# Iasonaspg/GPU-Randomized-Block-Lanczos

Hardware: AMD Instinct MI355X
Metric: RBL iters/sec + time-to-k=20 eigenpairs, n=1e7 nnz/row=100 b=32; 1/2/4/8 GPU (higher is better)
Workload: dtype f64

## Files before the change

gpu-randomized-block-lanczos_amd/csrc/kernels.hpp:

```cpp
#pragma once
#include "rbl_common.hpp"

namespace rbl {

struct Panels {
  static constexpr int kMax = 2;
  const double* ptr[kMax] = {nullptr, nullptr};
  int count = 0;
  int w = 0;
};
struct PanelRun {
  const double* base = nullptr;
  const float* base32 = nullptr;
  int64_t stride = 0;
  int count = 0;
  int w = 0;
};

constexpr int64_t kCsrPad = 256;
constexpr int64_t kRowPad = 16;
constexpr int64_t kRowPad32 = 32;

struct CsrDev {
  int64_t nrows = 0;
// ... 194 lines not shown
  double* beta = nullptr;
  double* bb = nullptr;
  double* rr = nullptr;
  int* iters = nullptr;
  int* status = nullptr;
  int* nactive = nullptr;
  double* hist = nullptr;
};
int cg_grid(int64_t nrows, int b);
void cg_resid(int64_t nrows, int b, const double* B, const double* W, const double* X, double sigma,
              double* R, double* part, double* dots, hipStream_t s);
void cg_dot(int64_t nrows, int b, const double* P, const double* W, double sigma, double* part,
            double* dots, hipStream_t s);
void cg_alpha(int b, const double* pap, const CgScalars& sc, hipStream_t s);
void cg_update(int64_t nrows, int b, double* X, double* R, const double* P, const double* W, double sigma,
               const CgScalars& sc, double* part, double* dots, hipStream_t s);
void cg_small(int rp, int b, const double* dv, const double* w, double* c, hipStream_t s);
void cg_beta(int b, int rp, bool init, int iter, const double* dots, const double* w, const double* c,
             double tol2, const CgScalars& sc, hipStream_t s);
void cg_dir(int64_t nrows, int b, int rp, const double* R, double* P, const double* V, const double* c,
            const CgScalars& sc, hipStream_t s);

constexpr int kKernRbf = 0, kKernLaplace = 1, kKernPoly = 2;
constexpr int kKernMaxDim = 256;
struct KernOp {
  int64_t n = 0;
  int d4 = 0;
  int kind = kKernRbf;
  int degree = 1;
  double gamma = 1.0, coef0 = 0.0, nugget = 0.0;
  const double* X = nullptr;
  const double* nrm = nullptr;
  const double* scale = nullptr;
};
void kernop_norms(int64_t n, int d4, const double* X, double* nrm, hipStream_t s);
bool kernop_apply(const KernOp& op, const double* Q, int b, double* U, hipStream_t s);

struct KernCross {
  int64_t mr = 0, mc = 0;
  int d4 = 0;
  int kind = kKernRbf;
  int degree = 1;
  double gamma = 1.0, coef0 = 0.0;
  const double* R = nullptr;
  const double* rnrm = nullptr;
  const double* C = nullptr;
  const double* cnrm = nullptr;
  const double* sr = nullptr;
  const double* sc = nullptr;
};
constexpr int kKernCrossWorkgroups = 512, kKernCrossMaxSplits = 64, kKernCrossMinStages = 4;
int kernop_cross_splits(int64_t mr, int64_t mc, int d4);
bool kernop_cross(const KernCross& op, const double* W, int b, double* Y, double* part, int splits,
                  hipStream_t s);

int gram_splits(int64_t nrows, int nW, int w, int xcols);
void gram_partial(int64_t nrows, const PanelRun& W, const Panels& X, double* slab, int splits,
                  const int* skip, hipStream_t s);
void reduce_slab(const double* slab, int splits, int64_t len, double* out, const int* skip,
                 hipStream_t s);
int reduce_scratch_splits(int splits);
void reduce_slab_many(double* slab, int splits, int64_t len, double* out, hipStream_t s);
void tsmm(int64_t nrows, const PanelRun& X, const double* C, int ldc, const Panels& Y,
          double alpha, double beta, const int* skip, hipStream_t s, double* xslab = nullptr,
          int* xgrid = nullptr);

constexpr int kCompressMaxCols = 512;
bool basis_compress_fast(const PanelRun& X, int p);
bool basis_compress(int64_t nrows, const PanelRun& X, const double* S_dev, int p, hipStream_t s,
                    bool generic = false);

bool gram44_ok(int64_t nrows, int nW, int w, int xcount, int xw);
int gram44_splits(int64_t nrows, int nW, int w = 32);
void gram44_partial(int64_t nrows, const PanelRun& W, const Panels& X, double* slab, int splits,
                    const int* skip, hipStream_t s);
bool tsmm44_ok(int xw, int ky, int yw);
void tsmm44_f32x(int64_t nrows, const PanelRun& X, const double* C, int ldc, const Panels& Y,
                 double alpha, double beta, hipStream_t s);
int tsmm44_xg_grid(int64_t nrows);
void tsmm44(int64_t nrows, const PanelRun& X, const double* C, int ldc, const Panels& Y,
            double alpha, double beta, const int* skip, hipStream_t s, double* xslab = nullptr,
            int* xgrid = nullptr);
bool tsmm44x32_ok(int64_t nrows, const PanelRun& X, const Panels& Y);
void tsmm44x32(int64_t nrows, const PanelRun& X, const double* C, int ldc, const Panels& Y,
               const int* skip, hipStream_t s);
int64_t tsmm44x32_shadow_slot(int64_t nrows);
void tsmm44x32_shadow(int64_t nrows, const PanelRun& X, const double* C, int ldc, const Panels& Y,
                      const int* skip, float* S, int nsh, int* cnt, hipStream_t s);
void shadow_block_rowmajor(const float* slot, int64_t nrows, float* out);

int gram32_splits(int64_t nrows);
void gram32_partial(int64_t nrows, const float* Wb, int64_t wstride, int nW, int w, const float* X0,
                    const float* X1, int xcount, double* slab, int splits, hipStream_t s);
void tsmm32(int64_t nrows, const float* Xb, int64_t xstride, int nX, int w, const double* C, int ldc,
            float* Y0, float* Y1, int ycount, float alpha, float beta, hipStream_t s);
void cvt_f32_to_f64(const float* src, double* dst, int64_t n, hipStream_t s);
void cvt_f64_to_f32(const double* src, float* dst, int64_t n, hipStream_t s);

void chol_step(const double* G, int b, int64_t nglobal, int mode, double* R, double* Rinv,
               double* Rtot, int* need3, int* status, const int* skip, hipStream_t s,
               double* scratch);
void copy_small(const double* src, double* dst, int64_t len, hipStream_t s, const int* skip = nullptr);
void cloc_rinv(double* C, const double* Rinv, int b, const int* skip, hipStream_t s);
void cloc_rinv2(double* C, const double* R1inv, const double* R2inv, int b, hipStream_t s);
void cloc_gate(const double* R, const double* Rinv, int b, const int* need3, double tau, int* gate,
               hipStream_t s);
void upd32_gate(const double* C, int K, int ncols, double tau, int force, int* flags, double* g_out,
                hipStream_t s);
void cloc_sub(double* G, const double* D, int nW, int b, hipStream_t s);
void transpose_small(const double* src, double* dst, int b, hipStream_t s);
void stash_step(const double* Ai, const double* Rtot, double* Bprev, int* flags, double* stash,
                int b, hipStream_t s);

struct RmatParams {
  int64_t n = 0;
  int scale = 0;
  int64_t edges = 0;
  double a = 0.57, b = 0.19, c = 0.19;
  uint64_t seed = 0;
  bool relabel = false;
  Scatter perm;
};
constexpr uint64_t kRelabelK = 0x52454C4142454C31ull;
void rmat_degree(const RmatParams& p, int32_t* deg, hipStream_t s);
int rmat_local_csr(const RmatParams& p, int64_t r0, int64_t r1, int64_t max_keys, int nplant,
                   const double* plant_dev, int64_t* rowptr_dev, int32_t** col_dev,
                   double** val_dev, int64_t* nnz_out, hipStream_t s);
void col_footprint(const int32_t* col, int64_t nnz, const int64_t* bounds_dev, int P,
                   unsigned long long* lo, unsigned long long* hi, hipStream_t s);

void circ_count(int64_t n, int64_t width, double p, uint64_t seed, int64_t r0, int64_t r1,
                int32_t* counts, hipStream_t s);
void circ_fill(int64_t n, int64_t width, double p, uint64_t seed, int64_t r0, int64_t r1,
               const int64_t* rowptr, int nplant, const double* plant_dev, int32_t* col,
               double* val, hipStream_t s);
void gather_rows(const double* Q, const int32_t* idx, int64_t nrows, int b, double* out,
                 hipStream_t s);
void mark_cols(const int32_t* col, int64_t nnz, int64_t r0, int64_t r1, uint8_t* mark,
               hipStream_t s);
void remap_cols(int32_t* col, int64_t nnz, const int32_t* map, hipStream_t s);
void hw_count(int64_t n, int64_t W, double p, uint64_t seed, int64_t r0, int64_t r1,
              int32_t* counts, hipStream_t s);
void hw_fill(int64_t n, int64_t W, double p, uint64_t seed, int64_t r0, int64_t r1,
             const int64_t* rowptr, int nplant, const double* plant_dev, int32_t* col,
             double* val, hipStream_t s);
void randn_block(double* Q, int64_t nrows, int b, int64_t r0, uint64_t seed, hipStream_t s,
                 const Scatter* perm = nullptr);
void tile_col_range(const CsrDev& A, int tile_rows, int64_t* cmin, int64_t* cmax, hipStream_t s);
void colmajor_to_rowmajor(const double* src, int64_t nrows, int w, double* dst, hipStream_t s);
void rowmajor_to_colmajor(const double* src, int64_t nrows, int w, double* dst, hipStream_t s);

}
```

gpu-randomized-block-lanczos_amd/csrc/rbl_api.cpp:

```cpp
#include <hip/hip_runtime.h>
#include <rocprofiler-sdk-roctx/roctx.h>

#include <algorithm>
#include <cstdlib>
#include <chrono>
#include <cmath>
#include <cstdio>
#include <cstring>
#include <string>
#include <thread>
#include <vector>

#include "../../include/rbl_hip.h"
#include "comm.hpp"
#include "kernels.hpp"

using namespace rbl;

namespace rbl::api {

template <class T>
struct DevBuf {
  T* p = nullptr;
  DevBuf() = default;
// ... 73 lines not shown
  DevBuf<int32_t> d_panel_blk;
  DevBuf<uint16_t> d_panel_cnt;
  DevBuf<uint32_t> d_panel_st;
  DevBuf<uint8_t> d_panel_col;
  DevBuf<double> d_panel_val;
};

struct SegTableBufs {
  DevBuf<int64_t> d_seg_trow;
  DevBuf<int32_t> d_seg_tinfo;
  DevBuf<int64_t> d_seg_slot_k0;
  DevBuf<int64_t> d_seg_lrow;
  DevBuf<int64_t> d_seg_lslot;
  DevBuf<double> d_seg_scratch;
};

struct TierBufs {
  SegTierBuf seg_tier[3];
  DevBuf<int32_t> d_send_idx;
  SegTierBuf push_tier;
  DevBuf<int64_t> d_ps_rows;
  DevBuf<int64_t> d_ps_ptr;
  DevBuf<int64_t> d_ps_slot;
};

struct RectShiftBufs {
  DevBuf<double> d_shift_u;
  DevBuf<double> d_shift_v;
  DevBuf<double> d_rect_ts;
  DevBuf<double> d_rect_part;
};

struct LowrankBufs {
  DevBuf<double> d_lr_P;
  DevBuf<double> d_lr_S;
  DevBuf<double> d_lr_wc;
  DevBuf<double> d_lr_part;
};

struct PrecondBufs {
  DevBuf<double> d_pc_V;
  DevBuf<double> d_pc_dv;
};

struct MatrixBufs : PanelBufs, SegTableBufs, TierBufs, RectShiftBufs, LowrankBufs, PrecondBufs {
  DevBuf<int64_t> d_rowptr;
  DevBuf<int32_t> d_col;
  DevBuf<double> d_val;
  DevBuf<int64_t> d_tcmin;
  DevBuf<int64_t> d_tcmax;
  DevBuf<int64_t> d_tinfo;
  DevBuf<uint16_t> d_bpos;
  DevBuf<double> d_bt;
  DevBuf<uint64_t> d_btp_hdr;
  DevBuf<double> d_bth;
  DevBuf<double> d_bte;
  DevBuf<double> d_btp_val;
  DevBuf<double> d_zrow;
  DevBuf<double> d_dense;
  DevBuf<double> d_qfull;
  SegTierBuf rect_side[2];
  DevBuf<double> d_rect_y;
  DevBuf<double> d_kern_x;
  DevBuf<double> d_kern_nrm;
  DevBuf<double> d_kern_scale;
};

struct RunBufs {
  DevBuf<double> d_basis;
  std::vector<PinBuf<char>> h_spill;
  DevBuf<double> d_stage;
  DevBuf<float> d_basis32;
  DevBuf<float> d_stage32;
  DevBuf<double> d_Qi64;
  DevBuf<double> d_Qm64;
  DevBuf<double> d_U;
  DevBuf<double> d_T;
  DevBuf<double> d_qext;
  DevBuf<double> d_sendbuf;
  DevBuf<double> d_pushbuf;
  DevBuf<double> d_precv;
  DevBuf<double> d_slab;
  DevBuf<double> d_C;
  DevBuf<double> d_small;
  DevBuf<int> d_flags;
  PinBuf<double> h_pin;
  PinBuf<double> h_hist;
  DevBuf<double> d_stash;
  DevBuf<double> d_lock;
  DevBuf<double> d_arrow_W;
  DevBuf<double> d_tr_S;
  DevBuf<double> d_filt[3];
  DevBuf<double> d_rv;
  DevBuf<double> d_rw;
  DevBuf<float> d_shadow;
};

struct CtxBufs {
  PinBuf<char> h_d2h[2];
  DevBuf<int> d_upd32;
  DevBuf<double> d_upd32_g;
};

}

struct rbl_ctx : rbl::api::MatrixBufs, rbl::api::RunBufs, rbl::api::CtxBufs {
  int device = 0;
  hipStream_t stream = nullptr;
  int nranks = 1, rank = 0;
  rbl::Comm* comm = nullptr;
  std::string err;

  int64_t n = 0, r0 = 0, r1 = 0, nloc = 0, nnz = 0;
  int64_t panel_nblk = 0;
  int panel_rpg = 4;
  int panel_ch = 48;
  bool panel_auto = false;
  int64_t panel_span = 0;
  int bt_ng = 0;
  int64_t seg_ntasks = 0, seg_nlong = 0;
  int seg_ntiers = 0;
  bool seg_split = false;
  bool ghost = false;
  int64_t n_ghost = 0, n_send = 0;
  std::vector<int64_t> ghost_cnt, ghost_off, send_cnt, send_off;
  const double* ghost_local = nullptr;
  bool ghost_active = false;
  bool halo_overlap = true;
  int halo_push_opt = 2;
  bool push = false;
  int64_t push_rows = 0;
  int64_t n_ps_rows = 0;
  size_t push_cap = 0;
  int64_t push_pred_rows = 0, pull_pred_rows = 0;
  hipEvent_t ev_push_ready = nullptr, ev_push_done = nullptr;
  hipStream_t hstream = nullptr;
  hipEvent_t ev_qready = nullptr, ev_halo = nullptr;
  bool dense = false;
  int64_t dense_panels = 0;
  int qfull_cols = 0;
  bool rect = false;
  int64_t rect_m = 0;
  int rect_y_cols = 0;
  bool rect_shift = false;
  int rect_ts_cols = 0;
  bool kernop = false;
  int kern_d = 0, kern_d4 = 0, kern_kind = 0, kern_degree = 0;
  double kern_gamma = 0.0, kern_coef0 = 0.0, kern_nugget = 0.0;
  int lr_r = 0, lr_rp = 0;
  int lr_cols = 0;
  int pc_r = 0, pc_rp = 0;
  int64_t ntiles = 0, tiles_per_wg = 0;
  bool window_ok16 = false, window_ok32 = false;
  bool band_ok16 = false, band_ok32 = false;
  bool band_gram = false;
  bool band_pair = false;
  std::vector<int64_t> bounds;
  std::vector<int64_t> need_lo, need_hi;
  std::vector<int64_t> give_lo, give_hi;
  int64_t ext_lo = 0, ext_hi = 0;
  bool split_halo = true;
  bool keep_csr = true;
  int relabel_opt = 0;
  bool relabeled = false;
  rbl::Scatter relabel_perm;
  bool csr_dropped = false;
// ... 1375 lines not shown
  const double c = 0.5 * (ctx->ser_lo + ctx->ser_hi), e = 0.5 * (ctx->ser_hi - ctx->ser_lo);
  const double* t1 = X;
  const double* t2 = nullptr;
  const int64_t len = ctx->nloc * b;
  for (int j = 1; j <= d; ++j) {
    double* tj = F[j % 3];
    const int st = apply_A(ctx, t1, 0, b, tj, nullptr, nullptr, nullptr);
    if (st < 0) return st;
    const double al = (j == 1 ? 1.0 : 2.0) / e;
    cheb_series_term(len, tj, t1, t2, al, -al * c, mu[j], mu[0], tj, out, j == 1, j == d, ctx->stream);
    HIPC(hipGetLastError());
    t2 = t1;
    t1 = tj;
  }
  return RBL_OK;
}

int filter_apply(rbl_ctx* ctx, const double* X, int b, double* out, const DevBuf<double> F[3]) {
  if (has_series(ctx)) return series_apply(ctx, X, b, out, F);
  return cheb_apply(ctx, X, b, out, F[0], F[1]);
}

constexpr double kUpd32Tau = 0.5;
constexpr int kUpd32Log = 64;

int lock_reorth(rbl_ctx* ctx, double* X) {
  const int b = ctx->b;
  for (int j = 0; j < ctx->nlock; ++j) {
    const double* l = ctx->d_lock + (int64_t)j * ctx->nloc;
    CHK(gram(ctx, run1(l, 1), pan1(X, b), ctx->d_C, nullptr));
    CHK(tsmm_checked(ctx, run1(l, 1), ctx->d_C, b, pan1(X, b), -1.0, 1.0, nullptr));
  }
  return RBL_OK;
}

bool cloc_derive_on(const rbl_ctx* ctx) {
  return ctx->cloc_derive && ctx->basis_bits == 64 && rowgram_ok(ctx->b) && (ctx->fuse & 3) == 3 &&
         ctx->reorth_order == 0 && !spilled(ctx) && (ctx->nranks == 1 || ctx->plan_all_resident);
}

int reorth_pair(rbl_ctx* ctx, int i, int flags) {
  const int b = ctx->b;
  double* Qi = slotp(ctx, i - 1);
  double* Qm = i >= 2 ? slotp(ctx, i - 2) : nullptr;
  shadow_written(ctx, i - 2);
  if ((flags & 2) && ctx->nlock > 0) {
    StageScope t(ctx, RBL_STAGE_PART_REORTH);
    if (Qm) CHK(lock_reorth(ctx, Qm));
    CHK(lock_reorth(ctx, Qi));
  }
  if ((flags & 1) && i >= 3) {
    StageScope t(ctx, RBL_STAGE_PART_REORTH);
    const int nW = i - 2;
    const int nres = std::min(nW, ctx->resident);
    const bool derive = cloc_derive_on(ctx) && b == 32 && ctx->cloc_step == i && !ctx->cloc_final &&
                        !((flags & 2) && ctx->nlock > 0) && nres == nW;
    const bool xg = (ctx->fuse & 2) && b == 32 && !derive;
    const int xg_parts = tsmm44_xg_grid(ctx->nloc);
    const bool xslab_ok = (size_t)(xg_parts + reduce_scratch_splits(xg_parts)) * b * b <= ctx->slab_elems;
    int xgrid = 0;
    auto update = [&](const PanelRun& W, bool last) -> int {
      const bool here = xg && last && xslab_ok;
      return tsmm_checked(ctx, W, ctx->d_C, 2 * b, pan2(Qi, Qm, b), -1.0, 1.0, nullptr,
                          here ? ctx->d_slab : nullptr, here ? &xgrid : nullptr);
    };
    if (ctx->reorth_order == 0) {
      PanelRun W;
      W.base = slotp(ctx, 0);
      W.stride = ctx->slot;
      W.count = nres;
      W.w = b;
      CHK(gram(ctx, W, pan2(Qi, Qm, b), ctx->d_C, nullptr));
      const Panels Yp = pan2(Qi, Qm, b);
      const bool gate32 = ctx->upd32 != 0 && b == 32 && !xg && nres == nW && !((flags & 2) && ctx->nlock > 0);
      const bool u32 = gate32 && ctx->nloc > 0 && tsmm44x32_ok(ctx->nloc, W, Yp);
      if (gate32) {
        upd32_gate(ctx->d_C, nW * b, 2 * b, kUpd32Tau, ctx->upd32 == 2, ctx->d_upd32,
                   ctx->d_upd32_g + (i % kUpd32Log), ctx->stream);
        HIPC(hipGetLastError());
      }
      if (u32) {
        if (ctx->d_shadow && ctx->shadow_opt && nW <= ctx->max_blocks - 2) {
          tsmm44x32_shadow(ctx->nloc, W, ctx->d_C, 2 * b, Yp, ctx->d_upd32, ctx->d_shadow,
                           ctx->shadow_valid, ctx->d_upd32 + 4, ctx->stream);
          ctx->shadow_valid = nW;
        } else {
          tsmm44x32(ctx->nloc, W, ctx->d_C, 2 * b, Yp, ctx->d_upd32, ctx->stream);
        }
        HIPC(hipGetLastError());
        CHK(tsmm_checked(ctx, W, ctx->d_C, 2 * b, Yp, -1.0, 1.0, ctx->d_upd32 + 1));
      } else {
        CHK(update(W, nres == nW));
      }
    } else {
      for (int j = 0; j < nres; ++j) {
        const PanelRun W = run1(slotp(ctx, j), b);
        CHK(gram(ctx, W, pan2(Qi, Qm, b), ctx->d_C, nullptr));
        CHK(update(W, j == nW - 1));
      }
    }
    for (int j = nres; j < nW; ++j) {
      int st = 0;
      const double* Wj = block_dev(ctx, j, i, &st);
      if (st) return fail(ctx, st, "partial reorth: H2D of a spilled block failed");
      CHK(gram(ctx, run1(Wj, b), pan2(Qi, Qm, b), ctx->d_C, nullptr));
      CHK(update(run1(Wj, b), j == nW - 1));
    }
    if (xg) {
      if (xgrid > 0) {
        reduce_slab_many(ctx->d_slab, xgrid, (int64_t)b * b, smallp(ctx, S_CLOC), ctx->stream);
      } else if (ctx->nloc > 0) {
        const int sp = gram_splits(ctx->nloc, 1, b, b);
        gram_partial(ctx->nloc, run1(Qm, b), pan1(Qi, b), ctx->d_slab, sp, nullptr, ctx->stream);
        reduce_slab(ctx->d_slab, sp, (int64_t)b * b, smallp(ctx, S_CLOC), nullptr, ctx->stream);
      } else {
        HIPC(hipMemsetAsync(smallp(ctx, S_CLOC), 0, (size_t)b * b * sizeof(double), ctx->stream));
      }
      HIPC(hipGetLastError());
      CHK(allreduce(ctx, smallp(ctx, S_CLOC), (size_t)b * b));
      ctx->cloc_step = i;
      ctx->cloc_final = true;
      ctx->cloc_src = 0;
    }
    if (derive) {
      cloc_sub(smallp(ctx, S_CLOC), ctx->d_C, nW, b, ctx->stream);
      HIPC(hipGetLastError());
      ctx->cloc_final = true;
      ctx->cloc_src = 2;
    }
  }
  return RBL_OK;
}

int combine_blocks(rbl_ctx* ctx, int nblocks, int kcols, const double* d_S, double* Y) {
  const int b = ctx->b;
  const int nres = std::min(nblocks, ctx->resident);
  PanelRun X;
  X.base = slotp(ctx, 0);
  X.stride = ctx->slot;
  X.count = nres;
  X.w = b;
  CHK(tsmm_checked(ctx, X, d_S, kcols, pan1(Y, kcols), 1.0, 0.0, nullptr));
  for (int j = nres; j < nblocks; ++j) {
    int st = 0;
    const double* Qj = block_dev(ctx, j, ctx->nblocks, &st);
    if (st) return fail(ctx, st, "Ritz: H2D of a spilled block failed");
    CHK(tsmm_checked(ctx, run1(Qj, b), d_S + (int64_t)j * b * kcols, kcols, pan1(Y, kcols), 1.0,
                     1.0, nullptr));
  }
  return RBL_OK;
}

int basis_combine(rbl_ctx* ctx, int nblocks, int kcols, const double* S, double* Y) {
  const int b = ctx->b;
  const int64_t rows = (int64_t)nblocks * b;
  DevBuf<double> d_Scm, d_S;
  HIPC(d_Scm.alloc(rows * kcols));
  HIPC(d_S.alloc(rows * kcols));
  HIPC(hipMemcpyAsync(d_Scm, S, rows * kcols * sizeof(double), hipMemcpyHostToDevice, ctx->stream));
  colmajor_to_rowmajor(d_Scm, rows, kcols, d_S, ctx->stream);
  const int st = combine_blocks(ctx, nblocks, kcols, d_S, Y);
  HIPC(hipStreamSynchronize(ctx->stream));
  return st;
}

int combine_blocks32(rbl_ctx* ctx, int nblocks, int kcols, const double* d_S, double* Y) {
  const int b = ctx->b;
  if (ctx->nloc <= 0) return RBL_OK;
  const int nres = std::min(nblocks, ctx->resident);
  int j0 = 0;
// ... 1663 lines not shown
  HIPC(hipSetDevice(ctx->device));
  HIPC(hipStreamSynchronize(ctx->stream));
  int dev_slots = max_blocks + 1;
  const bool same_shape = (ctx->d_basis || ctx->d_basis32) && ctx->b == b &&
                          ctx->max_blocks == max_blocks && ctx->slot == ctx->nloc * b &&
                          ctx->basis_bits == basis_bits;
  const int cur_slots = ctx->resident == INT32_MAX ? ctx->max_blocks + 1 : ctx->resident + 2;
  if (ctx->dev_blocks_opt < 0 && same_shape && ctx->auto_planned) {
    dev_slots = cur_slots;
  } else if (ctx->dev_blocks_opt != 0) {
    int g = ctx->dev_blocks_opt;
    if (g < 0) {
      size_t fr = 0, tot = 0;
      HIPC(hipMemGetInfo(&fr, &tot));
      const double blk64 = (double)std::max<int64_t>(ctx->nloc, 1) * b * 8.0;
      const double blk = blk64 * (basis_bits == 64 ? 1.0 : 0.5);
      const double mine = ctx->d_basis ? (double)(ctx->resident == INT32_MAX ? ctx->max_blocks + 1 : ctx->resident + 2) * blk64
                        : ctx->d_basis32 ? (double)(ctx->resident == INT32_MAX ? ctx->max_blocks + 1 : ctx->resident + 2) * blk64 * 0.5
                        : 0.0;
      const double mine_all = mine + (double)ctx->shadow_bytes;
      const double work = 2.0 + (ctx->nranks > 1 ? 1.0 : 0.0) +
                          (basis_bits == 32 ? 1.0 + (direct32_ok(ctx, b) ? 0.0 : 1.0) : 0.0);
      const double other = work * blk64 + blk + 8.0 * (double)gram_slab_elems(ctx, b, max_blocks, basis_bits);
      g = (int)std::max(3.0, std::floor((0.8 * ((double)fr + mine_all) - other) / blk));
    }
    dev_slots = std::min(dev_slots, std::max(3, g));
  }
  const bool reuse = same_shape && cur_slots == dev_slots;
  ctx->plan_all_resident = ctx->dev_blocks_opt == 0;
  ctx->nlock = 0;
  ctx->arrow_kb = 0;
  ctx->cloc_step = 0;
  ctx->shadow_valid = 0;
  ctx->step_flags.clear();
  const int alloc_st = [&]() -> int {
  if (reuse) {
    ctx->nblocks = 0;
    if (ctx->cstream) HIPC(hipStreamSynchronize(ctx->cstream));
    ctx->d2h_pending[0] = ctx->d2h_pending[1] = false;
    HIPC(hipMemsetAsync(ctx->d_flags, 0, 4 * sizeof(int), ctx->stream));
  } else {
  free_run(ctx);
  ctx->b = b;
  ctx->max_blocks = max_blocks;
  ctx->slot = ctx->nloc * b;
  const int64_t nl = std::max<int64_t>(ctx->nloc, 1);
  ctx->basis_bits = basis_bits;
  ctx->auto_planned = ctx->dev_blocks_opt < 0;
  if (basis_bits == 64) {
    HIPC(ctx->d_basis.alloc((size_t)dev_slots * nl * b));
    if (dev_slots < max_blocks + 1) {
      ctx->resident = dev_slots - 2;
      ctx->h_spill = std::vector<PinBuf<char>>(max_blocks + 1 - ctx->resident);
      HIPC(ctx->d_stage.alloc((size_t)nl * b));
      CHK(ensure_spill_stream(ctx));
    }
  } else {
    const size_t len32 = ((size_t)dev_slots * nl + kRowPad32) * b;
    HIPC(ctx->d_basis32.alloc(len32));
    HIPC(hipMemsetAsync(ctx->d_basis32, 0, len32 * sizeof(float), ctx->stream));
    if (dev_slots < max_blocks + 1) {
      ctx->resident = dev_slots - 2;
      ctx->h_spill = std::vector<PinBuf<char>>(max_blocks + 1 - ctx->resident);
      HIPC(ctx->d_stage32.alloc(((size_t)nl + kRowPad32) * b));
      HIPC(hipMemsetAsync(ctx->d_stage32, 0, ((size_t)nl + kRowPad32) * b * sizeof(float), ctx->stream));
      CHK(ensure_spill_stream(ctx));
    }
    HIPC(ctx->d_Qi64.alloc((nl + kRowPad) * b));
    if (!direct32_ok(ctx, b)) HIPC(ctx->d_Qm64.alloc((nl + kRowPad) * b));
  }
  HIPC(ctx->d_U.alloc((nl + kRowPad) * b));
  ctx->T_cols = b;
  HIPC(ctx->d_T.alloc(nl * b));
  if (ctx->nranks > 1) {
    CHK(ensure_qext(ctx, b, ctx->stream));
    if (ctx->ghost)
      HIPC(ctx->d_sendbuf.alloc(std::max<int64_t>(ctx->n_send, 1) * b));
  }
  const size_t slab = gram_slab_elems(ctx, b, max_blocks, basis_bits);
  ctx->slab_elems = slab;
  HIPC(ctx->d_slab.alloc(slab));
  ctx->C_elems = (size_t)std::max(1, max_blocks) * b * 2 * b;
  HIPC(ctx->d_C.alloc(ctx->C_elems));
  HIPC(ctx->d_small.alloc((size_t)S_NSMALL * b * b));
  HIPC(hipMemset(ctx->d_small, 0, (size_t)S_NSMALL * b * b * sizeof(double)));
  HIPC(ctx->d_flags.alloc(6));
  HIPC(hipMemset(ctx->d_flags, 0, 6 * sizeof(int)));
  if (!ctx->d_upd32) {
    HIPC(ctx->d_upd32.alloc(6));
    HIPC(hipMemset(ctx->d_upd32, 0, 6 * sizeof(int)));
    HIPC(ctx->d_upd32_g.alloc(kUpd32Log));
    HIPC(hipMemset(ctx->d_upd32_g, 0, kUpd32Log * sizeof(double)));
  }
  {
#ifdef RBL_VARIANTS
    const char* e = std::getenv("RBL_STASH_COPY");
    ctx->stash_direct = !(e && std::atoi(e) == 1);
#else
    ctx->stash_direct = true;
#endif
    const unsigned hf = ctx->stash_direct ? (hipHostMallocMapped | hipHostMallocCoherent) : hipHostMallocDefault;
    HIPC(ctx->h_pin.alloc(stash_rec(b), hf));
    HIPC(ctx->h_hist.alloc((size_t)(max_blocks + 2) * stash_rec(b), hf));
    if ((size_t)ctx->nloc * b * sizeof(double) >= 4 * kD2HPiece && !d2h_direct()) {
      CHK(ensure_d2h_slots(ctx));
      CHK(ensure_ritz_stream(ctx));
    }
    if (ctx->stash_direct) {
      HIPC(hipHostGetDevicePointer(reinterpret_cast<void**>(&ctx->dv_pin), ctx->h_pin, 0));
      HIPC(hipHostGetDevicePointer(reinterpret_cast<void**>(&ctx->dv_hist), ctx->h_hist, 0));
    } else {
      HIPC(ctx->d_stash.alloc(stash_rec(b)));
    }
  }
  if (ctx->shadow_opt && ctx->upd32 != 0 && basis_bits == 64 && b == 32 && !spilled(ctx) &&
      max_blocks >= 3 && ctx->nloc > 0) {
    const int64_t sslot = tsmm44x32_shadow_slot(ctx->nloc);
    const size_t need = (size_t)(max_blocks - 2) * (size_t)sslot * sizeof(float);
    size_t fr = 0, tot = 0;
    if (hipMemGetInfo(&fr, &tot) == hipSuccess && rbl_plan_shadow_fits(fr, tot, need)) {
      if (ctx->d_shadow.alloc((size_t)(max_blocks - 2) * (size_t)sslot) == hipSuccess) {
        ctx->shadow_slot = sslot;
        ctx->shadow_bytes = need;
      } else {
        (void)hipGetLastError();
      }
    }
  }
  }
  if (ctx->push && ctx->nranks > 1 && use_ghost(ctx, b)) {
    const char* inj = std::getenv("RBL_FAULT_PUSH_ALLOC");
    if (inj && *inj && std::atoi(inj) == ctx->rank)
      return fail(ctx, RBL_ERR_OOM, "rbl_start: push buffers (injected by RBL_FAULT_PUSH_ALLOC)");
    CHK(ensure_push(ctx, b));
  }
  if (has_filter(ctx)) CHK(ensure_filter_bufs(ctx, b));
  return RBL_OK;
  }();
  if (ctx->nranks > 1) {
    const int64_t mine = alloc_st;
    std::vector<int64_t> all(ctx->nranks);
    COMMC(ctx->comm->allgather_host(&mine, all.data(), 1, ctx->stream, &ctx->err));
    int bad = -1;
    for (int q = 0; q < ctx->nranks && bad < 0; ++q)
      if (all[q] != RBL_OK) bad = q;
    if (bad >= 0) {
      (void)hipGetLastError();
      free_run(ctx);
      if (alloc_st != RBL_OK) return alloc_st;
      return fail(ctx, (int)all[bad], "rbl_start: rank " + std::to_string(bad) +
                                          " could not allocate its run buffers");
    }
  } else if (alloc_st != RBL_OK) {
    (void)hipGetLastError();
    return alloc_st;
  }

  if (omega) {
    double* d_tmp = ctx->d_U;
    HIPC(hipMemcpyAsync(d_tmp, omega, ctx->nloc * b * sizeof(double), hipMemcpyHostToDevice,
                        ctx->stream));
    colmajor_to_rowmajor(d_tmp, ctx->nloc, b, ctx->d_T, ctx->stream);
  } else {
    randn_block(ctx->d_T, ctx->nloc, b, ctx->r0, seed, ctx->stream,
                ctx->relabeled ? &ctx->relabel_perm : nullptr);
  }
// ... 1724 lines not shown
```

gpu-randomized-block-lanczos_amd/csrc/reorth.hip:

```cpp
#include <algorithm>
#include <cstdlib>

#include "kernels.hpp"

namespace rbl {

__device__ __forceinline__ double mfma4(double a, double b, double c) {
  return __builtin_amdgcn_mfma_f64_4x4x4f64(a, b, c, 0, 0, 0);
}
#ifndef RBL_REORTH_ABL
#define RBL_REORTH_ABL 0
#endif
#ifndef RBL_REORTH_NT
#define RBL_REORTH_NT 0
#endif
template <typename T>
__device__ __forceinline__ T ldw(const T* p) {
  if constexpr (RBL_REORTH_NT) return __builtin_nontemporal_load(p);
  return *p;
}

constexpr int kG44Waves = 4;
#ifndef RBL_G44_ROWS
#define RBL_G44_ROWS 16
// ... 696 lines not shown
      mfmas(ch, acur);
      if (!(RBL_REORTH_ABL & 4)) store_c((ch + 1) & 1, cr);
#pragma unroll
      for (int rt = 0; rt < NRT; ++rt)
#pragma unroll
        for (int h = 0; h < NH; ++h) acur[rt][h] = anext[rt][h];
      if (!(RBL_REORTH_ABL & 2)) __syncthreads();
    }
  }
  double* ot = cs_raw + wave * 16 * KYP;
  const int g = (lane >> 2) & 3;
  constexpr int kYPer = 16 * KYP / 128;
  constexpr int kRowStep = 128 / KYP;
  const int ce = (2 * lane) % KYP, rl = (2 * lane) / KYP;
  const int yt = ce >= Y.w ? 1 : 0;
  double* yb = const_cast<double*>(yt ? Y.ptr[Panels::kMax - 1] : Y.ptr[0]) + (ce - yt * Y.w) +
               (rw + rl) * Y.w;
  const int dskip = (int)(r0 - rw);
  const bool has_beta = beta != 0.0;
#pragma unroll
  for (int rt = 0; rt < NRT; ++rt) {
    if constexpr (GL) {
#pragma unroll
      for (int cp = 0; cp < CG / 2; ++cp)
        *reinterpret_cast<d2v*>(ot + (4 * g + q) * KYP + ((8 * cp + 2 * (lane & 3)) ^ (4 * g))) =
            d2v{alpha * acc[rt][2 * cp], alpha * acc[rt][2 * cp + 1]};
    } else {
#pragma unroll
      for (int cg = 0; cg < CG; ++cg)
        ot[(4 * g + q) * KYP + ((4 * cg + (lane & 3)) ^ (4 * g))] = alpha * acc[rt][cg];
    }
#pragma unroll
    for (int m = 0; m < kYPer; ++m) {
      const int row = rl + kRowStep * m;
      d2v v = *reinterpret_cast<const d2v*>(ot + row * KYP + (ce ^ (4 * ((row >> 2) & 3))));
      const bool own = 16 * rt + row >= dskip;
      if (own) {
        d2v* yp = reinterpret_cast<d2v*>(yb + (int64_t)((16 * rt + kRowStep * m) * Y.w));
        if (has_beta) v += beta * *yp;
        *yp = v;
      }
      if constexpr (XG)
        *reinterpret_cast<d2v*>(ot + row * KYP + (ce ^ (4 * ((row >> 2) & 3)))) = own ? v : d2v{0.0, 0.0};
    }
    if constexpr (XG) {
      const int li = lane & 15;
#pragma unroll
      for (int s4 = 0; s4 < 4; ++s4) {
        const double* orow = ot + (4 * s4 + q) * KYP;
        double za[NT], yb[NT];
#pragma unroll
        for (int t2 = 0; t2 < NT; ++t2) {
          za[t2] = orow[(YW + 16 * t2 + li) ^ (4 * s4)];
          yb[t2] = orow[(16 * t2 + li) ^ (4 * s4)];
        }
#pragma unroll
        for (int it = 0; it < NT; ++it)
#pragma unroll
          for (int jt = 0; jt < NT; ++jt)
            gx[it][jt] = __builtin_amdgcn_mfma_f64_16x16x4f64(za[it], yb[jt], gx[it][jt], 0, 0, 0);
      }
    }
  }
  if constexpr (XG) {
    __syncthreads();
    const int li = lane & 15;
    constexpr int G2 = YW * YW;
    double* gw = cs_raw + wave * G2;
#pragma unroll
    for (int it = 0; it < NT; ++it)
#pragma unroll
      for (int jt = 0; jt < NT; ++jt)
#pragma unroll
        for (int reg = 0; reg < 4; ++reg) gw[(16 * it + q + 4 * reg) * YW + 16 * jt + li] = gx[it][jt][reg];
    __syncthreads();
    double* out = xslab + tile * G2;
    for (int e = tid; e < G2; e += 256)
      out[e] = (cs_raw[e] + cs_raw[G2 + e]) + (cs_raw[2 * G2 + e] + cs_raw[3 * G2 + e]);
  }
  };
  tile_body(blockIdx.x);
}

typedef float f2v32 __attribute__((ext_vector_type(2)));
typedef float f4v32 __attribute__((ext_vector_type(4)));
constexpr int kU32Rows = 32;
__host__ __device__ inline int64_t shadow_slot_floats(int64_t nrows) { return (nrows + 31) / 32 * 1024; }
template <bool SH>
__global__ __launch_bounds__(256) void k_tsmm44x32(int64_t nrows, PanelRun X,
                                                   const double* __restrict__ C, int ldc, double* Y0,
                                                   double* Y1, const int* skip, float* S, int nsh,
                                                   int* cnt) {
  constexpr int W = 32, KYP = 64, CT = 4, CLD = 64, KF = 32, NH = KF / 8, OLD = KYP + 4;
  const bool skipped = skip && *skip;
  if (!SH && skipped) return;
  __shared__ __attribute__((aligned(16))) float cs[2][KF * CLD + 128];
  static_assert(2 * (KF * CLD + 128) >= 4 * 16 * OLD, "epilogue tiles fit");
  const int tid = threadIdx.x, lane = tid & 63;
  const int wave = __builtin_amdgcn_readfirstlane(tid >> 6);
  const int q = lane >> 4, c16 = lane & 15;
  const int64_t r0 = ((int64_t)blockIdx.x * 4 + wave) * kU32Rows;
  const int64_t rw = r0 + kU32Rows <= nrows ? r0 : nrows - kU32Rows;
  const int nch = X.count;

  f4v32 acc[2][CT];
#pragma unroll
  for (int rt = 0; rt < 2; ++rt)
#pragma unroll
    for (int c = 0; c < CT; ++c) acc[rt][c] = f4v32{0.f, 0.f, 0.f, 0.f};

  const unsigned aoff0 = (unsigned)(c16 * W + 2 * q);
  auto load_a = [&](int ch, d2v (&ar)[2][NH]) {
    const int chc = ch < nch ? ch : nch - 1;
    const double* xb = X.base + (int64_t)chc * X.stride + rw * W;
#pragma unroll
    for (int h = 0; h < NH; ++h)
#pragma unroll
      for (int rt = 0; rt < 2; ++rt)
        ar[rt][h] = *reinterpret_cast<const d2v*>(xb + (aoff0 + (unsigned)(16 * rt * W + 8 * h)));
  };
  auto round_a = [&](const d2v (&ar)[2][NH], float (&af)[2][NH][2]) {
#pragma unroll
    for (int rt = 0; rt < 2; ++rt)
#pragma unroll
      for (int h = 0; h < NH; ++h) {
        af[rt][h][0] = (float)ar[rt][h].x;
        af[rt][h][1] = (float)ar[rt][h].y;
      }
  };
  const int ck = tid >> 4, ccc = tid & 15;
  auto load_c = [&](int ch, float (&cr)[2][CT]) {
    const int chc = ch < nch ? ch : nch - 1;
    const double* cb = C + (int64_t)(KF * chc + ck) * ldc + ccc;
#pragma unroll
    for (int hh = 0; hh < 2; ++hh)
#pragma unroll
      for (int ct = 0; ct < CT; ++ct) cr[hh][ct] = (float)cb[(int64_t)(16 * hh) * ldc + 16 * ct];
  };
  auto store_c = [&](int buf, const float (&cr)[2][CT]) {
#pragma unroll
    for (int hh = 0; hh < 2; ++hh)
      *reinterpret_cast<f4v32*>(&cs[buf][(ck + 16 * hh) * CLD + 4 * ccc]) =
          f4v32{cr[hh][0], cr[hh][1], cr[hh][2], cr[hh][3]};
  };

  const int64_t sslot = shadow_slot_floats(nrows);
  unsigned soff[2];
#pragma unroll
  for (int rt = 0; rt < 2; ++rt) {
    const int64_t r = rw + 16 * rt + c16;
    soff[rt] = (unsigned)((r >> 5) * 1024 + (((r >> 4) & 1) * 128 + 16 * q + (r & 15)) * 4);
  }
  auto load_s = [&](int ch, d2v (&ar)[2][NH]) {
    const float* sb = S + (int64_t)ch * sslot;
#pragma unroll
    for (int rt = 0; rt < 2; ++rt)
#pragma unroll
      for (int hf = 0; hf < 2; ++hf)
        ar[rt][hf] = __builtin_bit_cast(d2v, *reinterpret_cast<const f4v32*>(sb + (soff[rt] + 256u * hf)));
  };
  auto take_s = [&](const d2v (&ar)[2][NH], float (&af)[2][NH][2]) {
#pragma unroll
    for (int rt = 0; rt < 2; ++rt)
#pragma unroll
      for (int h = 0; h < NH; ++h) {
        const f4v32 sr = __builtin_bit_cast(f4v32, ar[rt][h >> 1]);
        af[rt][h][0] = sr[2 * (h & 1)];
        af[rt][h][1] = sr[2 * (h & 1) + 1];
      }
  };
  auto store_s = [&](int ch, const float (&af)[2][NH][2]) {
    float* sb = S + (int64_t)ch * sslot;
#pragma unroll
    for (int rt = 0; rt < 2; ++rt)
#pragma unroll
      for (int hf = 0; hf < 2; ++hf)
        *reinterpret_cast<f4v32*>(sb + (soff[rt] + 256u * hf)) =
            f4v32{af[rt][2 * hf][0], af[rt][2 * hf][1], af[rt][2 * hf + 1][0], af[rt][2 * hf + 1][1]};
  };

  d2v anext[2][NH];
  float af[2][NH][2];
  float cr[2][CT];
  if constexpr (SH) {
    if (blockIdx.x == 0 && tid == 0) {
      cnt[0] += skipped ? 0 : nsh;
      cnt[1] += nch - nsh;
    }
    if (skipped) {
      for (int ch = nsh; ch < nch; ++ch) {
        load_a(ch, anext);
        round_a(anext, af);
        store_s(ch, af);
      }
      return;
    }
  }
  load_c(0, cr);
  store_c(0, cr);
  if (SH && nsh > 0) {
    load_s(0, anext);
    take_s(anext, af);
  } else {
    load_a(0, anext);
    round_a(anext, af);
    if constexpr (SH) store_s(0, af);
  }
  __syncthreads();
  for (int ch = 0; ch < nch; ++ch) {
    load_c(ch + 1, cr);
    const bool ns = SH && ch + 1 < nsh;
    if (ns) load_s(ch + 1, anext);
    else load_a(ch + 1, anext);
    const float* cb = cs[ch & 1] + 2 * q * CLD + 4 * c16;
#pragma unroll
    for (int hv = 0; hv < 2 * NH; ++hv) {
      const int h = hv >> 1, v = hv & 1;
      const f4v32 bv = *reinterpret_cast<const f4v32*>(cb + (8 * h + v) * CLD);
#pragma unroll
      for (int rt = 0; rt < 2; ++rt)
#pragma unroll
        for (int c = 0; c < CT; ++c)
          acc[rt][c] = __builtin_amdgcn_mfma_f32_16x16x4f32(af[rt][h][v], bv[c], acc[rt][c], 0, 0, 0);
    }
    store_c((ch + 1) & 1, cr);
    if (ns) {
      take_s(anext, af);
    } else {
      round_a(anext, af);
      if constexpr (SH)
        if (ch + 1 < nch) store_s(ch + 1, af);
    }
    __syncthreads();
  }
  float* ot = &cs[0][0] + wave * 16 * OLD;
  const int ce = (2 * lane) % KYP, rl = (2 * lane) / KYP;
  double* yb = (ce < W ? Y0 + ce : Y1 + (ce - W)) + (rw + rl) * W;
  const int dskip = (int)(r0 - rw);
#pragma unroll
  for (int rt = 0; rt < 2; ++rt) {
#pragma unroll
    for (int c = 0; c < CT; ++c)
#pragma unroll
      for (int v = 0; v < 4; ++v) ot[(4 * q + v) * OLD + 16 * c + c16] = acc[rt][c][v];
    __builtin_amdgcn_wave_barrier();
    __builtin_amdgcn_fence(__ATOMIC_RELEASE, "wavefront");
#pragma unroll
    for (int m = 0; m < 8; ++m) {
      const int row = rl + 2 * m;
      const f2v32 p = *reinterpret_cast<const f2v32*>(ot + row * OLD + ce);
      if (16 * rt + row >= dskip) {
        d2v* yp = reinterpret_cast<d2v*>(yb + (int64_t)((16 * rt + 2 * m) * W));
        d2v y = *yp;
        y.x -= (double)p.x;
        y.y -= (double)p.y;
        *yp = y;
      }
    }
    __builtin_amdgcn_fence(__ATOMIC_ACQUIRE, "wavefront");
    __builtin_amdgcn_wave_barrier();
  }
}

bool tsmm44x32_ok(int64_t nrows, const PanelRun& X, const Panels& Y) {
  if (X.w != 32 || X.count < 1 || !X.base || Y.count != 2 || Y.w != 32 || nrows < kU32Rows) return false;
  for (int t = 0; t < Y.count; ++t)
    if (Y.ptr[t] >= X.base && Y.ptr[t] < X.base + (int64_t)X.count * X.stride) return false;
  return true;
}

void tsmm44x32(int64_t nrows, const PanelRun& X, const double* C, int ldc, const Panels& Y,
               const int* skip, hipStream_t st) {
  const int64_t wgs = (nrows + 4 * kU32Rows - 1) / (4 * kU32Rows);
  hipLaunchKernelGGL(k_tsmm44x32<false>, dim3((unsigned)wgs), dim3(256), 0, st, nrows, X, C, ldc,
                     const_cast<double*>(Y.ptr[0]), const_cast<double*>(Y.ptr[1]), skip, nullptr, 0, nullptr);
}

int64_t tsmm44x32_shadow_slot(int64_t nrows) { return shadow_slot_floats(nrows); }

void tsmm44x32_shadow(int64_t nrows, const PanelRun& X, const double* C, int ldc, const Panels& Y,
                      const int* skip, float* S, int nsh, int* cnt, hipStream_t st) {
  const int64_t wgs = (nrows + 4 * kU32Rows - 1) / (4 * kU32Rows);
  hipLaunchKernelGGL(k_tsmm44x32<true>, dim3((unsigned)wgs), dim3(256), 0, st, nrows, X, C, ldc,
                     const_cast<double*>(Y.ptr[0]), const_cast<double*>(Y.ptr[1]), skip, S,
                     std::min(std::max(nsh, 0), X.count), cnt);
}

void shadow_block_rowmajor(const float* slot, int64_t nrows, float* out) {
  for (int64_t r = 0; r < nrows; ++r)
    for (int k = 0; k < 32; ++k) {
      const int h = k >> 3, q = (k & 7) >> 1, v = k & 1;
      const int64_t f4 = (r >> 5) * 256 + ((r >> 4) & 1) * 128 + (h >> 1) * 64 + 16 * q + (r & 15);
      out[r * 32 + k] = slot[f4 * 4 + 2 * (h & 1) + v];
    }
}

bool tsmm44_ok(int xw, int ky, int yw) {
  return (xw == 16 || xw == 32) && ky >= 1 && ky <= 64 && yw % 2 == 0;
}

template <int B, int KYP, bool F32X = false>
static void launch_tsmm44(int64_t nrows, const PanelRun& X, const double* C, int ldc, int KY,
                          const Panels& Y, double alpha, double beta, const int* skip,
                          hipStream_t st) {
  const int64_t wgs = (nrows + 4 * kT44Rows - 1) / (4 * kT44Rows);
  hipLaunchKernelGGL((k_tsmm44<B, KYP, F32X>), dim3((unsigned)wgs), dim3(256), 0, st, nrows, X, C,
                     ldc, KY, Y, alpha, beta, skip);
}

void tsmm44_f32x(int64_t nrows, const PanelRun& X, const double* C, int ldc, const Panels& Y,
                 double alpha, double beta, hipStream_t st) {
  const int KY = Y.count * Y.w;
  if (X.w == 32) {
    if (KY <= 16) return launch_tsmm44<32, 16, true>(nrows, X, C, ldc, KY, Y, alpha, beta, nullptr, st);
    if (KY <= 32) return launch_tsmm44<32, 32, true>(nrows, X, C, ldc, KY, Y, alpha, beta, nullptr, st);
    return launch_tsmm44<32, 64, true>(nrows, X, C, ldc, KY, Y, alpha, beta, nullptr, st);
  }
  if (KY <= 16) return launch_tsmm44<16, 16, true>(nrows, X, C, ldc, KY, Y, alpha, beta, nullptr, st);
  if (KY <= 32) return launch_tsmm44<16, 32, true>(nrows, X, C, ldc, KY, Y, alpha, beta, nullptr, st);
  return launch_tsmm44<16, 64, true>(nrows, X, C, ldc, KY, Y, alpha, beta, nullptr, st);
}

int tsmm44_xg_grid(int64_t nrows) {
  return (int)((nrows + 4 * kT44fRows - 1) / (4 * kT44fRows));
}

void tsmm44(int64_t nrows, const PanelRun& X, const double* C, int ldc, const Panels& Y,
            double alpha, double beta, const int* skip, hipStream_t st, double* xslab, int* xgrid) {
  if (xgrid) *xgrid = 0;
  const int KY = Y.count * Y.w;
#ifdef RBL_VARIANTS
  static const bool fast_ok = [] {
    const char* e = getenv("RBL_TSMM44_FAST");
    return !e || atoi(e) != 0;
  }();
#else
  constexpr bool fast_ok = true;
#endif
  bool alias = false;
  for (int t = 0; t < Y.count; ++t)
    alias |= Y.ptr[t] >= X.base && Y.ptr[t] < X.base + (int64_t)X.count * X.stride;
#ifdef RBL_VARIANTS
  static const bool fast32 = [] {
    const char* e = getenv("RBL_TSMM44_FAST32");
    return e && atoi(e) != 0;
  }();
#else
  constexpr bool fast32 = false;
#endif
  if (fast_ok && (KY == 64 || (KY == 32 && fast32)) && (X.count * X.w) % kT44K == 0 &&
      nrows >= kT44fRows && Y.w % 2 == 0 && !alias) {
    const int64_t wgs = (nrows + 4 * kT44fRows - 1) / (4 * kT44fRows);
    const bool xg = xslab && KY == 64 && Y.count == 2 && 2 * Y.w == KY;
    if (xg) *xgrid = (int)wgs;
    const bool gl = RBL_T44_GLDS && RBL_T44_PF == 1 && ldc % 2 == 0 &&
                    reinterpret_cast<uintptr_t>(C) % 16 == 0;
#define RBL_T44F(BB, XGG, KK)                                                                      \
  do {                                                                                              \
    if (gl)                                                                                         \
      hipLaunchKernelGGL((k_tsmm44f<BB, RBL_T44_KC, RBL_T44_PF, XGG, KK, RBL_T44_GLDS && RBL_T44_PF == 1>), \
                         dim3((unsigned)wgs), dim3(256), 0, st, nrows, X, C, ldc, Y, alpha, beta, skip, \
                         XGG ? xslab : nullptr);                                                    \
    else                                                                                            \
      hipLaunchKernelGGL((k_tsmm44f<BB, RBL_T44_KC, RBL_T44_PF, XGG, KK, false>), dim3((unsigned)wgs), \
                         dim3(256), 0, st, nrows, X, C, ldc, Y, alpha, beta, skip, XGG ? xslab : nullptr); \
  } while (0)
    if (KY == 64) {
      if (X.w == 32) { if (xg) RBL_T44F(32, true, 64); else RBL_T44F(32, false, 64); }
// ... 23 lines not shown
```

Measured before the change: 55.77.

## Use split-bf16 MFMA with pre-split C staged via LDS DMA in fp32 reorth update

```diff
diff --git a/gpu-randomized-block-lanczos_amd/csrc/kernels.hpp b/gpu-randomized-block-lanczos_amd/csrc/kernels.hpp
--- a/gpu-randomized-block-lanczos_amd/csrc/kernels.hpp
+++ b/gpu-randomized-block-lanczos_amd/csrc/kernels.hpp
@@ -300,11 +300,12 @@
             double alpha, double beta, const int* skip, hipStream_t s, double* xslab = nullptr,
             int* xgrid = nullptr);
 bool tsmm44x32_ok(int64_t nrows, const PanelRun& X, const Panels& Y);
+int64_t tsmm44x32_cpieces(int K);
 void tsmm44x32(int64_t nrows, const PanelRun& X, const double* C, int ldc, const Panels& Y,
-               const int* skip, hipStream_t s);
+               const int* skip, unsigned short* Cp, hipStream_t s);
 int64_t tsmm44x32_shadow_slot(int64_t nrows);
 void tsmm44x32_shadow(int64_t nrows, const PanelRun& X, const double* C, int ldc, const Panels& Y,
-                      const int* skip, float* S, int nsh, int* cnt, hipStream_t s);
+                      const int* skip, float* S, int nsh, int* cnt, unsigned short* Cp, hipStream_t s);
 void shadow_block_rowmajor(const float* slot, int64_t nrows, float* out);
 
 int gram32_splits(int64_t nrows);
diff --git a/gpu-randomized-block-lanczos_amd/csrc/rbl_api.cpp b/gpu-randomized-block-lanczos_amd/csrc/rbl_api.cpp
--- a/gpu-randomized-block-lanczos_amd/csrc/rbl_api.cpp
+++ b/gpu-randomized-block-lanczos_amd/csrc/rbl_api.cpp
@@ -179,6 +179,7 @@
   DevBuf<double> d_precv;
   DevBuf<double> d_slab;
   DevBuf<double> d_C;
+  DevBuf<unsigned short> d_C16;
   DevBuf<double> d_small;
   DevBuf<int> d_flags;
   PinBuf<double> h_pin;
@@ -1720,10 +1721,10 @@
       if (u32) {
         if (ctx->d_shadow && ctx->shadow_opt && nW <= ctx->max_blocks - 2) {
           tsmm44x32_shadow(ctx->nloc, W, ctx->d_C, 2 * b, Yp, ctx->d_upd32, ctx->d_shadow,
-                           ctx->shadow_valid, ctx->d_upd32 + 4, ctx->stream);
+                           ctx->shadow_valid, ctx->d_upd32 + 4, ctx->d_C16, ctx->stream);
           ctx->shadow_valid = nW;
         } else {
-          tsmm44x32(ctx->nloc, W, ctx->d_C, 2 * b, Yp, ctx->d_upd32, ctx->stream);
+          tsmm44x32(ctx->nloc, W, ctx->d_C, 2 * b, Yp, ctx->d_upd32, ctx->d_C16, ctx->stream);
         }
         HIPC(hipGetLastError());
         CHK(tsmm_checked(ctx, W, ctx->d_C, 2 * b, Yp, -1.0, 1.0, ctx->d_upd32 + 1));
@@ -3553,6 +3554,7 @@
   HIPC(ctx->d_slab.alloc(slab));
   ctx->C_elems = (size_t)std::max(1, max_blocks) * b * 2 * b;
   HIPC(ctx->d_C.alloc(ctx->C_elems));
+  if (b == 32) HIPC(ctx->d_C16.alloc((size_t)tsmm44x32_cpieces(std::max(1, max_blocks) * b)));
   HIPC(ctx->d_small.alloc((size_t)S_NSMALL * b * b));
   HIPC(hipMemset(ctx->d_small, 0, (size_t)S_NSMALL * b * b * sizeof(double)));
   HIPC(ctx->d_flags.alloc(6));
diff --git a/gpu-randomized-block-lanczos_amd/csrc/reorth.hip b/gpu-randomized-block-lanczos_amd/csrc/reorth.hip
--- a/gpu-randomized-block-lanczos_amd/csrc/reorth.hip
+++ b/gpu-randomized-block-lanczos_amd/csrc/reorth.hip
@@ -802,20 +802,66 @@
   tile_body(blockIdx.x);
 }
 
+#ifndef RBL_U32_BF16
+#define RBL_U32_BF16 1
+#endif
+#ifndef RBL_U32_WPE
+#define RBL_U32_WPE (RBL_U32_BF16 ? 3 : 4)
+#endif
+#ifndef RBL_U32_CDMA
+#define RBL_U32_CDMA 1
+#endif
 typedef float f2v32 __attribute__((ext_vector_type(2)));
 typedef float f4v32 __attribute__((ext_vector_type(4)));
+typedef __bf16 bf2v __attribute__((ext_vector_type(2)));
+typedef __bf16 bf8v __attribute__((ext_vector_type(8)));
 constexpr int kU32Rows = 32;
+__device__ __forceinline__ void split3_bf16(const float (&w)[8], bf8v (&p)[3]) {
+  float r[8];
+#pragma unroll
+  for (int j = 0; j < 8; ++j) r[j] = w[j];
+#pragma unroll
+  for (int s = 0; s < 3; ++s)
+#pragma unroll
+    for (int j = 0; j < 8; j += 2) {
+      const bf2v b = __builtin_convertvector(f2v32{r[j], r[j + 1]}, bf2v);
+      p[s][j] = b[0];
+      p[s][j + 1] = b[1];
+      if (s < 2) {
+        const f2v32 f = __builtin_convertvector(b, f2v32);
+        r[j] -= f[0];
+        r[j + 1] -= f[1];
+      }
+    }
+}
+constexpr int kU32CpChunk = 3 * 2048;
+__global__ __launch_bounds__(256) void k_upd32_split_c(const double* __restrict__ C, int ldc,
+                                                       unsigned short* __restrict__ Cp, const int* skip) {
+  if (skip && *skip) return;
+  const int tid = threadIdx.x;
+  const double* cb = C + (int64_t)(32 * blockIdx.x + 2 * (tid >> 6)) * ldc + (tid & 63);
+  float cr[8];
+#pragma unroll
+  for (int j = 0; j < 8; ++j) cr[j] = (float)cb[(int64_t)(8 * (j >> 1) + (j & 1)) * ldc];
+  bf8v cp[3];
+  split3_bf16(cr, cp);
+#pragma unroll
+  for (int p = 0; p < 3; ++p)
+    *reinterpret_cast<bf8v*>(Cp + (int64_t)blockIdx.x * kU32CpChunk + 2048 * p + 8 * tid) = cp[p];
+}
 __host__ __device__ inline int64_t shadow_slot_floats(int64_t nrows) { return (nrows + 31) / 32 * 1024; }
 template <bool SH>
-__global__ __launch_bounds__(256) void k_tsmm44x32(int64_t nrows, PanelRun X,
+__global__ __launch_bounds__(256) __attribute__((amdgpu_waves_per_eu(RBL_U32_WPE))) void k_tsmm44x32(int64_t nrows, PanelRun X,
                                                    const double* __restrict__ C, int ldc, double* Y0,
                                                    double* Y1, const int* skip, float* S, int nsh,
-                                                   int* cnt) {
+                                                   int* cnt, const unsigned short* __restrict__ Cp) {
   constexpr int W = 32, KYP = 64, CT = 4, CLD = 64, KF = 32, NH = KF / 8, OLD = KYP + 4;
+  constexpr bool BF = RBL_U32_BF16, CD = BF && RBL_U32_CDMA;
+  constexpr int CPC = KF * KYP / 2, CBUF = BF ? 3 * CPC : KF * CLD + 128;
   const bool skipped = skip && *skip;
   if (!SH && skipped) return;
-  __shared__ __attribute__((aligned(16))) float cs[2][KF * CLD + 128];
-  static_assert(2 * (KF * CLD + 128) >= 4 * 16 * OLD, "epilogue tiles fit");
+  __shared__ __attribute__((aligned(16))) float cs[2][CBUF];
+  static_assert(2 * CBUF >= 4 * 16 * OLD, "epilogue tiles fit");
   const int tid = threadIdx.x, lane = tid & 63;
   const int wave = __builtin_amdgcn_readfirstlane(tid >> 6);
   const int q = lane >> 4, c16 = lane & 15;
@@ -839,29 +885,44 @@
       for (int rt = 0; rt < 2; ++rt)
         ar[rt][h] = *reinterpret_cast<const d2v*>(xb + (aoff0 + (unsigned)(16 * rt * W + 8 * h)));
   };
-  auto round_a = [&](const d2v (&ar)[2][NH], float (&af)[2][NH][2]) {
+  auto round_a = [&](const d2v (&ar)[2][NH], float (&af)[2][8]) {
 #pragma unroll
     for (int rt = 0; rt < 2; ++rt)
 #pragma unroll
       for (int h = 0; h < NH; ++h) {
-        af[rt][h][0] = (float)ar[rt][h].x;
-        af[rt][h][1] = (float)ar[rt][h].y;
-      }
-  };
-  const int ck = tid >> 4, ccc = tid & 15;
-  auto load_c = [&](int ch, float (&cr)[2][CT]) {
+        af[rt][2 * h] = (float)ar[rt][h].x;
+        af[rt][2 * h + 1] = (float)ar[rt][h].y;
+      }
+  };
+  const int ck = BF ? 2 * (tid >> 6) : tid >> 4, ccc = BF ? tid & 63 : tid & 15;
+  auto load_c = [&](int ch, float (&cr)[8]) {
     const int chc = ch < nch ? ch : nch - 1;
     const double* cb = C + (int64_t)(KF * chc + ck) * ldc + ccc;
 #pragma unroll
-    for (int hh = 0; hh < 2; ++hh)
-#pragma unroll
-      for (int ct = 0; ct < CT; ++ct) cr[hh][ct] = (float)cb[(int64_t)(16 * hh) * ldc + 16 * ct];
-  };
-  auto store_c = [&](int buf, const float (&cr)[2][CT]) {
-#pragma unroll
-    for (int hh = 0; hh < 2; ++hh)
-      *reinterpret_cast<f4v32*>(&cs[buf][(ck + 16 * hh) * CLD + 4 * ccc]) =
-          f4v32{cr[hh][0], cr[hh][1], cr[hh][2], cr[hh][3]};
+    for (int j = 0; j < 8; ++j)
+      cr[j] = (float)cb[BF ? (int64_t)(8 * (j >> 1) + (j & 1)) * ldc
+                           : (int64_t)(16 * (j >> 2)) * ldc + 16 * (j & 3)];
+  };
+  auto store_c = [&](int buf, const float (&cr)[8]) {
+    if constexpr (BF) {
+      bf8v cp[3];
+      split3_bf16(cr, cp);
+#pragma unroll
+      for (int p = 0; p < 3; ++p) *reinterpret_cast<bf8v*>(&cs[buf][p * CPC + 4 * tid]) = cp[p];
+    } else {
+#pragma unroll
+      for (int hh = 0; hh < 2; ++hh)
+        *reinterpret_cast<f4v32*>(&cs[buf][(ck + 16 * hh) * CLD + 4 * ccc]) =
+            f4v32{cr[4 * hh], cr[4 * hh + 1], cr[4 * hh + 2], cr[4 * hh + 3]};
+    }
+  };
+  auto dma_c = [&](int buf, int ch) {
+    const int chc = ch < nch ? ch : nch - 1;
+    const unsigned short* src = Cp + (int64_t)chc * kU32CpChunk + 8 * tid;
+#pragma unroll
+    for (int p = 0; p < 3; ++p)
+      __builtin_amdgcn_global_load_lds((glb_vptr)(src + 2048 * p), (lds_vptr)(&cs[buf][p * CPC + 256 * wave]), 16,
+                                       0, 0);
   };
 
   const int64_t sslot = shadow_slot_floats(nrows);
@@ -879,29 +940,36 @@
       for (int hf = 0; hf < 2; ++hf)
         ar[rt][hf] = __builtin_bit_cast(d2v, *reinterpret_cast<const f4v32*>(sb + (soff[rt] + 256u * hf)));
   };
-  auto take_s = [&](const d2v (&ar)[2][NH], float (&af)[2][NH][2]) {
+  auto take_s = [&](const d2v (&ar)[2][NH], float (&af)[2][8]) {
 #pragma unroll
     for (int rt = 0; rt < 2; ++rt)
 #pragma unroll
-      for (int h = 0; h < NH; ++h) {
-        const f4v32 sr = __builtin_bit_cast(f4v32, ar[rt][h >> 1]);
-        af[rt][h][0] = sr[2 * (h & 1)];
-        af[rt][h][1] = sr[2 * (h & 1) + 1];
-      }
-  };
-  auto store_s = [&](int ch, const float (&af)[2][NH][2]) {
+      for (int hf = 0; hf < 2; ++hf) {
+        const f4v32 sr = __builtin_bit_cast(f4v32, ar[rt][hf]);
+#pragma unroll
+        for (int e = 0; e < 4; ++e) af[rt][4 * hf + e] = sr[e];
+      }
+  };
+  auto store_s = [&](int ch, const float (&af)[2][8]) {
     float* sb = S + (int64_t)ch * sslot;
 #pragma unroll
     for (int rt = 0; rt < 2; ++rt)
 #pragma unroll
       for (int hf = 0; hf < 2; ++hf)
         *reinterpret_cast<f4v32*>(sb + (soff[rt] + 256u * hf)) =
-            f4v32{af[rt][2 * hf][0], af[rt][2 * hf][1], af[rt][2 * hf + 1][0], af[rt][2 * hf + 1][1]};
+            f4v32{af[rt][4 * hf], af[rt][4 * hf + 1], af[rt][4 * hf + 2], af[rt][4 * hf + 3]};
   };
 
   d2v anext[2][NH];
-  float af[2][NH][2];
-  float cr[2][CT];
+  float af[2][8];
+  bf8v ap[2][3];
+  auto split_a = [&] {
+    if constexpr (BF) {
+#pragma unroll
+      for (int rt = 0; rt < 2; ++rt) split3_bf16(af[rt], ap[rt]);
+    }
+  };
+  float cr[8];
   if constexpr (SH) {
     if (blockIdx.x == 0 && tid == 0) {
       cnt[0] += skipped ? 0 : nsh;
@@ -916,8 +984,12 @@
       return;
     }
   }
-  load_c(0, cr);
-  store_c(0, cr);
+  if constexpr (CD) {
+    dma_c(0, 0);
+  } else {
+    load_c(0, cr);
+    store_c(0, cr);
+  }
   if (SH && nsh > 0) {
     load_s(0, anext);
     take_s(anext, af);
@@ -926,24 +998,44 @@
     round_a(anext, af);
     if constexpr (SH) store_s(0, af);
   }
+  split_a();
   __syncthreads();
+  constexpr int PA[6] = {0, 2, 1, 0, 1, 0}, PB[6] = {2, 0, 1, 1, 0, 0};
   for (int ch = 0; ch < nch; ++ch) {
-    load_c(ch + 1, cr);
+    if constexpr (CD) {
+      if (ch + 1 < nch) dma_c((ch + 1) & 1, ch + 1);
+    } else {
+      load_c(ch + 1, cr);
+    }
     const bool ns = SH && ch + 1 < nsh;
     if (ns) load_s(ch + 1, anext);
     else load_a(ch + 1, anext);
-    const float* cb = cs[ch & 1] + 2 * q * CLD + 4 * c16;
-#pragma unroll
-    for (int hv = 0; hv < 2 * NH; ++hv) {
-      const int h = hv >> 1, v = hv & 1;
-      const f4v32 bv = *reinterpret_cast<const f4v32*>(cb + (8 * h + v) * CLD);
-#pragma unroll
-      for (int rt = 0; rt < 2; ++rt)
-#pragma unroll
-        for (int c = 0; c < CT; ++c)
-          acc[rt][c] = __builtin_amdgcn_mfma_f32_16x16x4f32(af[rt][h][v], bv[c], acc[rt][c], 0, 0, 0);
-    }
-    store_c((ch + 1) & 1, cr);
+    if constexpr (BF) {
+      const float* cb = cs[ch & 1] + (64 * q + c16) * 4;
+#pragma unroll
+      for (int c = 0; c < CT; ++c) {
+        bf8v bp[3];
+#pragma unroll
+        for (int p = 0; p < 3; ++p) bp[p] = *reinterpret_cast<const bf8v*>(cb + p * CPC + 64 * c);
+#pragma unroll
+        for (int s = 0; s < 6; ++s)
+#pragma unroll
+          for (int rt = 0; rt < 2; ++rt)
+            acc[rt][c] = __builtin_amdgcn_mfma_f32_16x16x32_bf16(ap[rt][PA[s]], bp[PB[s]], acc[rt][c], 0, 0, 0);
+      }
+    } else {
+      const float* cb = cs[ch & 1] + 2 * q * CLD + 4 * c16;
+#pragma unroll
+      for (int j = 0; j < 8; ++j) {
+        const f4v32 bv = *reinterpret_cast<const f4v32*>(cb + (8 * (j >> 1) + (j & 1)) * CLD);
+#pragma unroll
+        for (int rt = 0; rt < 2; ++rt)
+#pragma unroll
+          for (int c = 0; c < CT; ++c)
+            acc[rt][c] = __builtin_amdgcn_mfma_f32_16x16x4f32(af[rt][j], bv[c], acc[rt][c], 0, 0, 0);
+      }
+    }
+    if constexpr (!CD) store_c((ch + 1) & 1, cr);
     if (ns) {
       take_s(anext, af);
     } else {
@@ -951,6 +1043,7 @@
       if constexpr (SH)
         if (ch + 1 < nch) store_s(ch + 1, af);
     }
+    split_a();
     __syncthreads();
   }
   float* ot = &cs[0][0] + wave * 16 * OLD;
@@ -989,21 +1082,33 @@
   return true;
 }
 
+int64_t tsmm44x32_cpieces(int K) { return (int64_t)(K / 32) * kU32CpChunk; }
+
+static void upd32_split_c(const PanelRun& X, const double* C, int ldc, const int* skip, unsigned short* Cp,
+                          hipStream_t st) {
+  constexpr bool kSplit = bool(RBL_U32_BF16) && bool(RBL_U32_CDMA);
+  if (kSplit)
+    hipLaunchKernelGGL(k_upd32_split_c, dim3((unsigned)X.count), dim3(256), 0, st, C, ldc, Cp, skip);
+}
+
 void tsmm44x32(int64_t nrows, const PanelRun& X, const double* C, int ldc, const Panels& Y,
-               const int* skip, hipStream_t st) {
+               const int* skip, unsigned short* Cp, hipStream_t st) {
   const int64_t wgs = (nrows + 4 * kU32Rows - 1) / (4 * kU32Rows);
+  upd32_split_c(X, C, ldc, skip, Cp, st);
   hipLaunchKernelGGL(k_tsmm44x32<false>, dim3((unsigned)wgs), dim3(256), 0, st, nrows, X, C, ldc,
-                     const_cast<double*>(Y.ptr[0]), const_cast<double*>(Y.ptr[1]), skip, nullptr, 0, nullptr);
+                     const_cast<double*>(Y.ptr[0]), const_cast<double*>(Y.ptr[1]), skip, nullptr, 0, nullptr,
+                     Cp);
 }
 
 int64_t tsmm44x32_shadow_slot(int64_t nrows) { return shadow_slot_floats(nrows); }
 
 void tsmm44x32_shadow(int64_t nrows, const PanelRun& X, const double* C, int ldc, const Panels& Y,
-                      const int* skip, float* S, int nsh, int* cnt, hipStream_t st) {
+                      const int* skip, float* S, int nsh, int* cnt, unsigned short* Cp, hipStream_t st) {
   const int64_t wgs = (nrows + 4 * kU32Rows - 1) / (4 * kU32Rows);
+  upd32_split_c(X, C, ldc, skip, Cp, st);
   hipLaunchKernelGGL(k_tsmm44x32<true>, dim3((unsigned)wgs), dim3(256), 0, st, nrows, X, C, ldc,
                      const_cast<double*>(Y.ptr[0]), const_cast<double*>(Y.ptr[1]), skip, S,
-                     std::min(std::max(nsh, 0), X.count), cnt);
+                     std::min(std::max(nsh, 0), X.count), cnt, Cp);
 }
 
 void shadow_block_rowmajor(const float* slot, int64_t nrows, float* out) {
```

After: 58.15, median of 6. 1.04x the previous value.
